# AgentFoundryExamples/lqr-quadcopter-test

Hardware: AMD Instinct MI355X
Metric: env-steps/sec at 65 536 parallel episodes per GPU (30 s @ dt=0.01, Riccati-LQR closed loop) (higher is better)
Workload: dtype f64; 1 GPU; BASELINE configs[1]: 65536 episodes/GPU x 3000 steps, linear target, Riccati-LQR shared K, RK4 dt=0.01; episodes_per_gpu=65536, episodes_total=65536, parallelism=episode-sharded x1

## Files before the change

lqr-quadcopter-test_amd/csrc/qt_device.hpp:

```cpp
#pragma once

#include <hip/hip_runtime.h>
#include <math.h>
#include <stdint.h>

#include "../../include/quadtrack.h"
#include "qt_glibc.hpp"
#include "qt_math.hpp"

namespace qt {

constexpr double kPi = 3.141592653589793;
constexpr double kTwoPi = 6.283185307179586;
constexpr double kMaxTilt = kPi / 3.0;

__device__ __forceinline__ double clipd(double v, double lo, double hi) {
  double r = v < lo ? lo : v;
  return r > hi ? hi : r;
}

__device__ __forceinline__ double dot3_blas(double a, double b, double c) { return fma(c, c, fma(b, b, a * a)); }
__device__ __forceinline__ double norm3(double a, double b, double c) { return sqrt(dot3_blas(a, b, c)); }

__device__ __forceinline__ bool same_sign(double a, double b) {
// ... 343 lines not shown
  double o[5];
  rk4_linear(delta, h, 1.0, zero, o);
  L.cv = o[3], L.pv = o[4];
  double sw = 0.0, sp = 0.0;
#pragma unroll
  for (int i = 0; i < 4; ++i) {
    double f[4] = {0.0, 0.0, 0.0, 0.0};
    f[i] = 1.0;
    rk4_linear(delta, h, 0.0, f, o);
    L.wv[i] = o[3];
    sw += o[3];
    if (i < 3) L.pa[i] = o[4], sp += o[4];
  }
  const double g = pl.gz * pl.inv_mass;
  L.gv = g * sw;
  L.gp = g * sp;
  return L;
}

struct Horizon {
  int on;
  double tmax;
  double vmax;
  double vmax2;
  double inv_2vmax;
  double vabs;
  double pmax;
  double pabs;
  double inv_dang;
  double inv_tstep;
  double slack;
  long long tie_exp_bits;
  int dual_below;
};

QT_HD Horizon make_horizon(const qt_env_params& e, const qt_ctrl_params& c, const RateLin& rl) {
  Horizon h{};
  const double tm = fmax(fabs(c.min_thrust), fabs(c.max_thrust));
  const bool ok = e.max_velocity > 1e-100 && e.max_velocity < 1e150 && e.max_position > 1e-100 &&
                  e.max_position < 1e150 && e.dt > 1e-100 && e.dt < 1e3 && fabs(e.max_episode_time) < 1e150 &&
                  tm < 1e150 && c.max_rate >= 0.0 && c.max_rate < 1e150;
  if (!ok) return h;
  h.on = 1;
  h.tmax = tm;
  h.vmax = e.max_velocity * (1.0 - 1e-12);
  h.vmax2 = h.vmax * h.vmax;
  h.inv_2vmax = 1.0 / (2.0 * h.vmax);
  h.vabs = e.max_velocity * 1e-14;
  h.pmax = e.max_position;
  h.pabs = e.max_position * 1e-15 + 1e-300;
  h.inv_dang = 1.0 / ((fabs(rl.ay) + fabs(rl.au)) * c.max_rate * (1.0 + 1e-9) + 2e-15);
  h.inv_tstep = 1.0 / ((e.dt + (fabs(e.max_episode_time) + e.dt) * 4.5e-16) * (1.0 + 1e-9));
  h.slack = 1.0 + 1e-9;
  {
    int q = 0;
    double m = frexp(e.dt, &q) * 9007199254740992.0;
    q -= 53;
    while (fmod(m, 2.0) == 0.0) m *= 0.5, ++q;
    const long long be = (long long)(q + 53) + 1023;
    h.tie_exp_bits = (be > 0 && be < 2047) ? (be << 52) : -1;
  }
  return h;
}

struct LaunchConst {
  RateLin rl;
  VelLin vl;
  Plant pl;
  Horizon hz;
  double rc[5][3], rs[5][3];
  double om[5][3];
  unsigned long long* defer_flag;
  unsigned long long epoch;
  double* reward;
  const double* fresh_off;
  double* met;
};

QT_HD int pattern_omegas(const qt_env_params& e, int motion, double* om) {
  if (motion == QT_MOTION_CIRCULAR) {
    om[0] = e.speed / e.radius;
    return 1;
  }
  if (motion == QT_MOTION_SINUSOIDAL) {
    om[0] = 2.0 * kPi * e.frequency;
    om[1] = 2.0 * kPi * (e.frequency * 1.3);
// ... 437 lines not shown
  return tl ? QT_TERM_TIME_LIMIT : (pb ? QT_TERM_POSITION_BOUNDS : QT_TERM_RUNNING);
}


template <int KC, bool KS>
struct Gains {
  static constexpr int kCount = KC == 3 ? 9 : (KS ? (KC == 9 ? 9 : 6) : 4 * KC);
  double k[kCount];
};

template <int KC>
__host__ __device__ constexpr int structured_index(int j) {
  constexpr int rows[9] = {0, 0, 1, 1, 2, 2, 0, 1, 2};
  constexpr int cols[9] = {2, 5, 1, 4, 0, 3, 8, 7, 6};
  return rows[j] * KC + cols[j];
}

struct FFLane {
  double vg[3], ag[3], vmax;
};

__host__ __device__ inline FFLane ff_uniform(const qt_ctrl_params& c) {
  if (!c.feedforward_enabled) return FFLane{{0.0, 0.0, 0.0}, {0.0, 0.0, 0.0}, INFINITY};
  return FFLane{{c.ff_velocity_gain[0], c.ff_velocity_gain[1], c.ff_velocity_gain[2]},
                {c.ff_acceleration_gain[0], c.ff_acceleration_gain[1], c.ff_acceleration_gain[2]},
                c.ff_max_velocity};
}

__device__ __forceinline__ double add_product_rn(double a, double b, double c) {
#pragma clang fp contract(off)
  return a + b * c;
}

template <int KC, bool FF, bool KS, bool FAST = false>
__device__ __forceinline__ bool compute_action(const qt_ctrl_params& c, const Gains<KC, KS>& G, double hover,
                                               const double* qp, const double* qv, const Target& tg,
                                               const FFLane& f, double* integ, double* u, double* diag = nullptr,
                                               double em_fast = 0.0) {
  double ep[3], ev[3], tv[3] = {tg.v[0], tg.v[1], tg.v[2]}, ffa[3] = {0, 0, 0}, ffv[3] = {0, 0, 0};
#pragma unroll
  for (int i = 0; i < 3; ++i) ep[i] = tg.p[i] - qp[i];
  if (FF) {
    double vm = norm3(tv[0], tv[1], tv[2]);
    if (vm > f.vmax) {
      double scl = f.vmax / vm;
#pragma unroll
      for (int i = 0; i < 3; ++i) tv[i] = tv[i] * scl;
    }
#pragma unroll
    for (int i = 0; i < 3; ++i) {
      ffv[i] = f.vg[i] * tv[i];
      tv[i] = (1.0 + f.vg[i]) * tv[i];
    }
    double ac[3] = {tg.a[0], tg.a[1], tg.a[2]};
    double am = norm3(ac[0], ac[1], ac[2]);
    if (am > c.ff_max_acceleration && am > 0) {
#pragma unroll
      for (int i = 0; i < 3; ++i) ac[i] = ac[i] / am * c.ff_max_acceleration;
    }
#pragma unroll
    for (int i = 0; i < 3; ++i) ffa[i] = f.ag[i] * ac[i];
  }
#pragma unroll
  for (int i = 0; i < 3; ++i) ev[i] = tv[i] - qv[i];
  const double s[6] = {ep[0], ep[1], ep[2], ev[0], ev[1], ev[2]};
  double uf[4];
  if (KC == 9) {
// ... 24 lines not shown
      uf[1] = (G.k[2] * s[1] + G.k[3] * s[4]) + G.k[7] * integ[1];
      uf[2] = (G.k[4] * s[0] + G.k[5] * s[3]) + G.k[8] * integ[0];
      uf[3] = 0.0;
    } else {
#pragma unroll
      for (int r = 0; r < 4; ++r) {
        double a = 0.0, b = 0.0;
#pragma unroll
        for (int j = 0; j < 6; ++j) a += G.k[r * KC + j] * s[j];
#pragma unroll
        for (int j = 0; j < 3; ++j) b += G.k[r * KC + 6 + j] * integ[j];
        uf[r] = a + b;
      }
    }
  } else if (KS) {
    uf[0] = G.k[0] * s[2] + G.k[1] * s[5];
    uf[1] = G.k[2] * s[1] + G.k[3] * s[4];
    uf[2] = G.k[4] * s[0] + G.k[5] * s[3];
    uf[3] = 0.0;
  } else {
#pragma unroll
    for (int r = 0; r < 4; ++r) {
      double a = 0.0;
#pragma unroll
      for (int j = 0; j < 6; ++j) a += G.k[r * KC + j] * s[j];
      uf[r] = a;
    }
  }
  const double raw0 = FF ? hover + uf[0] + ffa[2] : hover + uf[0];
  const double raw1 = FF ? uf[1] + -ffa[1] : uf[1];
  const double raw2 = FF ? uf[2] + ffa[0] : uf[2];
  const double raw3 = uf[3];
  u[0] = clip_num(raw0, c.min_thrust, c.max_thrust);
  u[1] = clip_num(raw1, -c.max_rate, c.max_rate);
  u[2] = clip_num(raw2, -c.max_rate, c.max_rate);
  u[3] = (KS && FAST) ? 0.0 : clip_num(raw3, -c.max_rate, c.max_rate);
  if (!FAST && any_lane(!isfinite((raw0 + raw1) + (raw2 + raw3)))) {
    u[0] = raw0 != raw0 ? raw0 : u[0];
    u[1] = raw1 != raw1 ? raw1 : u[1];
    u[2] = raw2 != raw2 ? raw2 : u[2];
    u[3] = raw3 != raw3 ? raw3 : u[3];
  }
  if (diag) {
#pragma unroll
    for (int i = 0; i < 6; ++i) diag[i] = s[i];
#pragma unroll
    for (int i = 0; i < 4; ++i) diag[6 + i] = uf[i];
#pragma unroll
    for (int i = 0; i < 3; ++i) diag[10 + i] = ffv[i], diag[13 + i] = ffa[i];
  }
  return (u[0] != raw0) || (u[1] != raw1) || (u[2] != raw2) || (u[3] != raw3);
}

template <bool FF, bool FAST = false>
__device__ __forceinline__ void compute_action_pid(const qt_ctrl_params& c, const double* g, double hover,
                                                   const double* qp, const double* qv, const Target& tg, double now,
                                                   const FFLane& f, double* integ, double* u,
                                                   double* diag = nullptr) {
  const double *kp = g, *ki = g + 3, *kd = g + 6;
  double ep[3], tv[3] = {tg.v[0], tg.v[1], tg.v[2]}, ffa[3] = {0, 0, 0}, ffv[3] = {0, 0, 0};
#pragma unroll
  for (int i = 0; i < 3; ++i) ep[i] = tg.p[i] - qp[i];
  const double last = integ[3];
  const bool none = (__double_as_longlong(last) & 0x7fffffffffffffffLL) > 0x7ff0000000000000LL;
  const double dt = none ? 0.0 : now - last;
  integ[3] = now;
  const double lim = c.integral_limit;
  if (FAST) {
// ... 64 lines not shown
```

lqr-quadcopter-test_amd/csrc/qt_kernels.hpp:

```cpp
#pragma once
#include <hip/hip_runtime.h>

#include <type_traits>

#include "qt_device.hpp"


#ifndef QT_ABLATE
#define QT_ABLATE 0
#endif
#define QT_ABL_METRICS 1
#define QT_ABL_CONSTRAIN 2
#define QT_ABL_TERMINATION 4
#define QT_ABL_CONTROLLER 8
#define QT_ABL_TARGET 16

#ifndef QT_CLOCK_STAMP
#define QT_CLOCK_STAMP 0
#endif

namespace qtk {

using namespace qt;

// ... 446 lines not shown
    if (ADVANCE) rotor_advance<QT_MOTION_CIRCULAR>(k, dtt, rs, rc);
    target_from_rotor<FF, QT_MOTION_CIRCULAR>(e, pt, rs, rc, tg);
  } else if (motion == QT_MOTION_FIGURE8 && !FF) {
    if (ADVANCE) rotor_advance<QT_MOTION_FIGURE8>(k, dtt, rs, rc);
    target_from_rotor<false, QT_MOTION_FIGURE8>(e, pt, rs, rc, tg);
  } else {
    target_state<FF, true>(e, motion, pt, t, tg);
  }
}

__device__ __forceinline__ void clamp_velocity(const qt_env_params& e, double* x) {
  const double s = dot3_blas(x[3], x[4], x[5]);
  if (norm_gt(s, e.max_velocity)) {
    const double vm = sqrt(s);
#pragma unroll
    for (int i = 3; i < 6; ++i) x[i] = x[i] / vm * e.max_velocity;
  }
}

__device__ __forceinline__ void tilt_clamp(double* x, Trig& ta) {
  double sm, cm;
  sincos_tilt(kMaxTilt, &sm, &cm);
#pragma unroll
  for (int i = 0; i < 2; ++i) {
    x[6 + i] = clip_num(x[6 + i], -kMaxTilt, kMaxTilt);
    ta.s[i] = clip_num(ta.s[i], -sm, sm);
    ta.c[i] = fmax(ta.c[i], cm);
  }
}

constexpr int kMaxHorizon = 62;
constexpr int kVotedBurst = 4;

template <bool TILT, bool BINADE>
__device__ __forceinline__ int yaw0_horizon(const qt_env_params& e, const Horizon& hz, const VelLin& lin,
                                            const Plant& pl, const double* x, double t, int rem) {
  const double tmi = hz.tmax * pl.inv_mass;
  const double sw = (fabs(lin.wv[0]) + fabs(lin.wv[1])) + (fabs(lin.wv[2]) + fabs(lin.wv[3]));
  const double spa = (fabs(lin.pa[0]) + fabs(lin.pa[1])) + fabs(lin.pa[2]);
  const double dv = fma(fma(tmi, sw, fabs(lin.gv)), hz.slack, hz.vabs);
  const double dp = fma(fma(fabs(lin.pv), hz.vmax, fma(tmi, spa, fabs(lin.gp))), hz.slack, hz.pabs);
  const double s = fma(x[5], x[5], fma(x[4], x[4], x[3] * x[3]));
  double h = (hz.vmax2 - s) * hz.inv_2vmax * __builtin_amdgcn_rcp(dv);
  h = fmin(h, (hz.pmax - fmax(fabs(x[0]), fmax(fabs(x[1]), fabs(x[2])))) * __builtin_amdgcn_rcp(dp));
  if (TILT) h = fmin(h, (kMaxTilt - fmax(fabs(x[6]), fabs(x[7]))) * hz.inv_dang);
  h = fmin(h, (e.max_episode_time - t) * hz.inv_tstep);
  bool bin_ok = true;
  if (BINADE) {
    const long long eb = __double_as_longlong(t) & 0x7ff0000000000000LL;
    h = fmin(h, (__longlong_as_double(eb + (1LL << 52)) - t) * hz.inv_tstep);
    bin_ok = t > 0.0 && eb != hz.tie_exp_bits;
  }
  h = fma(h, 1.0 - 1e-6, -1.0);
  const bool lane_ok = h >= 2.0 && lin.cv >= 0.0 && lin.cv <= 1.0 && bin_ok;
  const int hl = lane_ok ? (int)fmin(h, (double)kMaxHorizon) : 0;
  int H = 0;
#pragma unroll
  for (int bit = 32; bit >= 2; bit >>= 1)
    if (__builtin_amdgcn_ballot_w64(hl < H + bit) == 0) H += bit;
  const int rcap = (rem - 1) & ~1;
  return hz.on ? (H < rcap ? H : rcap) : 0;
}

constexpr int kDualBelow = 8;
#ifndef QT_GROUPED_DUAL
#define QT_GROUPED_DUAL 0
#endif

template <bool RIDE>
__device__ __forceinline__ void ride_target(const qt_env_params& e, bool still, Target& tg) {
  if constexpr (RIDE) {
#pragma unroll
    for (int i = 0; i < 3; ++i) {
      tg.p[i] = still ? e.center[i] : tg.p[i];
      tg.v[i] = still ? 0.0 : tg.v[i];
      tg.a[i] = still ? 0.0 : tg.a[i];
    }
  }
}

template <int MOTION, int KC, bool FF, bool KS, bool UNI, bool DUAL = false, bool RIDE = false>
__device__ __forceinline__ void run_yaw0(const qt_env_params& e, const qt_ctrl_params& c, const qt_criteria& cr,
                                         int motion, const Pattern& pt, const Plant& pl_lane, double hover,
                                         const Gains<KC, KS>& G, const FFLane& fl, double* x, double* integ,
                                         Target& tg, double& t, Acc& a, int nsteps, const LaunchConst& k,
                                         bool still = false) {
  constexpr bool kRotor = MOTION == QT_MOTION_CIRCULAR || MOTION == QT_MOTION_SINUSOIDAL ||
                          (MOTION == QT_MOTION_FIGURE8 && !FF);
  constexpr int kNeg = -(1 << 30);
  const Plant pl = UNI ? k.pl : pl_lane;
  const VelLin lin = UNI ? k.vl : make_vel_lin(e, pl_lane);
  const double R = cr.target_radius, eR = e.target_radius;
  const double vm2 = e.max_velocity * e.max_velocity * (1.0 - 1e-14);
  const double pos_up = nextafter(e.max_position, INFINITY);
  const int W = cr.overshoot_window;
  double rs[3] = {0.0, 0.0, 0.0}, rc[3] = {1.0, 1.0, 1.0};
  if constexpr (kRotor) {
    rotor_init<MOTION>(pt, t, rs, rc);
    target_from_rotor<FF, MOTION>(e, pt, rs, rc, tg);
  } else if constexpr (MOTION < 0) {
    rotor_init_rt<FF>(motion, pt, t, rs, rc);
    rotor_target_rt<FF, false>(e, k, motion, pt, t, 0.0, rs, rc, tg);
  } else {
    target_state<FF, true>(e, motion, pt, t, tg);
  }
  ride_target<RIDE>(e, still, tg);
  double err = sqrt_pos(sq3_ref(tg.p[0] - x[0], tg.p[1] - x[1], tg.p[2] - x[2]));
  Trig ta;
  trig_of<true>(x + 6, ta);
  int z = a.prev_on == 1 ? 1 : (a.os_streak >= 0 ? a.os_streak + 1 : kNeg);
  double cur = a.os_cur;
  int on_pre = a.on_pre, on_post = a.on_post, os_count = a.os_count;
  bool stepped = false;
  constexpr bool kTiltHorizon = KC != 9;
  constexpr bool kFold = kRotor && KC == 9;
  int s = 0;
  while (a.term == QT_TERM_RUNNING && s < nsteps) {
    const int s0 = s;
    int rem = nsteps - s0 > (1 << 29) ? (1 << 29) : nsteps - s0;
    RateCoef rk;
    auto step = [&](auto vote, auto clamp, const double* fc, const double* fs) -> bool {
      constexpr bool VOTE = decltype(vote)::value, CLAMP = decltype(clamp)::value;
      rk.pin();
      const double a0[2] = {x[6], x[7]};
      double u[4];
      if (QT_ABLATE & QT_ABL_CONTROLLER) {
        u[0] = hover, u[1] = u[2] = u[3] = 0.0;
      } else {
        if constexpr (KC == 3)
          compute_action_pid<FF, true>(c, G.k, hover, x, x + 3, tg, t, fl, integ, u);
        else
          compute_action<KC, FF, KS, true>(c, G, hover, x, x + 3, tg, fl, integ, u, nullptr, err);
      }
      if (!(QT_ABLATE & QT_ABL_METRICS)) {
        a.sum_e += err;
        a.sum_e2 = fma(err, err, a.sum_e2);
        a.max_e = fmax(a.max_e, err);
        const bool on = err <= R;
        on_pre += on;
        a.sum_u += sqrt_sum(fma(u[2], u[2], fma(u[1], u[1], u[0] * u[0])));
        const bool counted = on & (z > W);
        os_count += counted;
        a.os_max = counted ? fmax(a.os_max, cur) : a.os_max;
        cur = on ? err - R : fmax(cur, err - R);
        z = on ? 1 : z + 1;
      }
      double d4[2];
      Trig t4;
      integrate_yaw0(k.rl, lin, pl, ta, x, u, rk, d4, t4);
      const double t0 = t;
      t += e.dt;
      if (!(QT_ABLATE & QT_ABL_TARGET)) {
        if constexpr (kRotor) {
          if (VOTE || !kFold)
            rotor_advance<MOTION>(k, (t - t0) - e.dt, rs, rc);
          else
            rotor_turn<MOTION>(fc, fs, rs, rc);
          target_from_rotor<FF, MOTION>(e, pt, rs, rc, tg);
        } else if constexpr (MOTION < 0) {
          rotor_target_rt<FF, true>(e, k, motion, pt, t, (t - t0) - e.dt, rs, rc, tg);
        } else {
          target_state<FF, true>(e, motion, pt, t, tg);
        }
        ride_target<RIDE>(e, still, tg);
      }
      err = sqrt_pos(sq3_ref(x[0] - tg.p[0], x[1] - tg.p[1], x[2] - tg.p[2]));
      on_post += err <= eR;
      if (!(QT_ABLATE & QT_ABL_CONSTRAIN)) constrain_fast_apply<true>(e, x);
      attitude_trig_resid(x + 6, a0, d4, t4, ta);
      if ((VOTE || CLAMP || !kTiltHorizon) && !(QT_ABLATE & QT_ABL_CONSTRAIN)) tilt_clamp(x, ta);
      if constexpr (!VOTE) return false;
      --rem;
      double stop_m =
          fmax(fmax(fmax(fabs(x[0]), fmax(fabs(x[1]), fabs(x[2]))) - pos_up, (x[3] * x[3] + x[4] * x[4] + x[5] * x[5]) - vm2),
               fmax(t - e.max_episode_time, -(double)rem));
      return __builtin_amdgcn_ballot_w64(stop_m >= 0.0) != 0;
    };
    do {
      int H = yaw0_horizon<kTiltHorizon, kFold>(e, k.hz, lin, pl, x, t, rem);
      bool clamp_body = false;
      if constexpr (DUAL) {
        if (H < k.hz.dual_below) {
          const int H2 = yaw0_horizon<false, kFold>(e, k.hz, lin, pl, x, t, rem);
          if (H2 > H) H = H2, clamp_body = true;
        }
      }
      using F = std::false_type;
      using T = std::true_type;
      if constexpr (kFold) {
        double fc[3], fs[3];
        rotor_fold<MOTION>(k, ((t + e.dt) - t) - e.dt, fc, fs);
        for (int j = 4; j <= H; j += 4) {
          step(F{}, F{}, fc, fs);
          step(F{}, F{}, fc, fs);
          step(F{}, F{}, fc, fs);
          step(F{}, F{}, fc, fs);
        }
        if (H & 2) {
          step(F{}, F{}, fc, fs);
          step(F{}, F{}, fc, fs);
        }
      } else if (DUAL && clamp_body) {
        for (int j = 4; j <= H; j += 4) {
          step(F{}, T{}, nullptr, nullptr);
          step(F{}, T{}, nullptr, nullptr);
          step(F{}, T{}, nullptr, nullptr);
          step(F{}, T{}, nullptr, nullptr);
        }
        if (H & 2) {
          step(F{}, T{}, nullptr, nullptr);
          step(F{}, T{}, nullptr, nullptr);
        }
      } else {
        for (int j = 4; j <= H; j += 4) {
          step(F{}, F{}, nullptr, nullptr);
          step(F{}, F{}, nullptr, nullptr);
          step(F{}, F{}, nullptr, nullptr);
          step(F{}, F{}, nullptr, nullptr);
        }
        if (H & 2) {
          step(F{}, F{}, nullptr, nullptr);
          step(F{}, F{}, nullptr, nullptr);
        }
      }
      rem -= H;
      const int nv = H > 0 ? 0 : (k.hz.on ? kVotedBurst : (1 << 30));
      bool stop = false;
      for (int j = 0; j < nv && !stop; ++j) stop = step(std::true_type{}, std::false_type{}, nullptr, nullptr);
      if (stop) break;
    } while (true);
    const int ran = (nsteps - s0 > (1 << 29) ? (1 << 29) : nsteps - s0) - rem;
    s += ran;
    a.steps += ran;
    stepped = true;
    z = z <= 0 ? kNeg : z;
    if (!(QT_ABLATE & QT_ABL_CONSTRAIN)) clamp_velocity(e, x);
    a.term = (QT_ABLATE & QT_ABL_TERMINATION) ? (t >= e.max_episode_time ? QT_TERM_TIME_LIMIT : QT_TERM_RUNNING)
                                               : termination_fast(e, t, x);
  }
  if (stepped) {
    a.on_pre = on_pre, a.on_post = on_post, a.os_count = os_count;
    a.prev_on = z == 1 ? 1 : 0;
    a.os_streak = z >= 2 ? z - 1 : -1;
    a.os_cur = cur;
  }
}

template <int FLAVOR, int MOTION, int KC, bool FF, bool KS, bool UNI = false, bool FRESH = true, bool REC = true,
          int INTEG = -1, bool RIDE = false, bool PIN = true>
__device__ __forceinline__ void rollout_lane(const qt_env_params& e, const qt_ctrl_params& c, const qt_criteria& cr,
                                             const BatchDev& b, const qt_state& st, int nsteps,
                                             double* __restrict__ rec, int deferred, const LaunchConst& lc,
                                             int64_t slot) {
  const int64_t n = b.n, ep = episode_of(b, slot);
  const int motion = MOTION >= 0 ? MOTION : motion_of(b, e, ep);
  const bool still = RIDE && slot_motion(b, slot) == QT_MOTION_STATIONARY;
  Pattern pt = pattern_of(b, e, motion, ep);
  if (RIDE) pt.c0 = still ? 0.0 : pt.c0, pt.c1 = still ? 0.0 : pt.c1, pt.c2 = still ? 0.0 : pt.c2;
  const Plant pl = UNI ? lc.pl : make_plant(e, b.plant_mass ? b.plant_mass[ep] : e.mass);
  const double hover = UNI ? c.hover_thrust : (b.hover ? b.hover[ep] : c.hover_thrust);
  Gains<KC, KS> G;
  load_gains<KC, KS, UNI>(b, ep, G);
  const FFLane fl = FF ? ff_of(b, c, ep) : FFLane{};

  constexpr int NI = KC == 9 ? 3 : (KC == 3 ? 4 : 0);
  double x[12], integ[4] = {0, 0, 0, 0};
  Target tg;
  double t;
  Acc a;
  if (FRESH && lc.fresh_off) {
    target_state<true>(e, motion, pt, 0.0, tg);
#pragma unroll
    for (int i = 0; i < 3; ++i) x[i] = tg.p[i] + lc.fresh_off[i * n + ep];
#pragma unroll
    for (int i = 3; i < 12; ++i) x[i] = 0.0;
    if (KC == 3) integ[3] = __longlong_as_double(0x7ff8000000000000LL);
    t = 0.0;
    a = Acc{0, 0, -INFINITY, 0, 0, 0, 0, 0, 0, -1, -1, 0, 0, QT_TERM_RUNNING};
  } else {
#pragma unroll
    for (int i = 0; i < 12; ++i) x[i] = st.x[i * n + ep];
#pragma unroll
// ... 23 lines not shown
      st.target[(6 + i) * n + ep] = tg.a[i];
    }
    st.t[ep] = t;
    store_acc(st.acc, n, ep, a);
  };

  bool lane_ok = a.term != QT_TERM_RUNNING ||
                 (all_finite(G.k, Gains<KC, KS>::kCount) && all_finite(x, 12) && all_finite(integ, 3) &&
                  all_finite(tg.p, 3) && all_finite(tg.v, 3) && all_finite(tg.a, 3) && finite_bits(hover) &&
                  (!FF || (all_finite(fl.vg, 3) && all_finite(fl.ag, 3) && !(fl.vmax < 0.0))) &&
                  finite_bits(pl.inv_mass) && finite_bits(t) && fabs(t) < 1e300);
  for (int i = 9; i < 12; ++i) lane_ok = lane_ok && fabs(x[i]) <= e.max_angular_velocity;
  if (FLAVOR == kExact && b.nseg && b.motion) lane_ok = lane_ok && (int)b.motion[ep] == slot_motion(b, slot);
  if (b.seg_check >= 0 && b.motion) lane_ok = lane_ok && (int)b.motion[ep] == b.seg_check;
  if (FLAVOR == kYaw0 || deferred == kYaw0)
    lane_ok = lane_ok && x[8] == 0.0 && x[11] == 0.0 && fabs(x[6]) <= kMaxTilt && fabs(x[7]) <= kMaxTilt &&
              fabs(x[9]) <= c.max_rate && fabs(x[10]) <= c.max_rate;
  const bool wave_ok = __builtin_amdgcn_ballot_w64(!lane_ok) == 0;
  if (FLAVOR != kExact) {
    if (!wave_ok) {
      if (lc.defer_flag) *lc.defer_flag = lc.epoch;
      if (FRESH && lc.fresh_off) store_state();
      return;
    }
    const bool rw = FRESH && lc.reward && a.term == QT_TERM_RUNNING;
    if (rw) lc.reward[ep] += a.sum_e + sqrt_pos(sq3_ref(tg.p[0] - x[0], tg.p[1] - x[1], tg.p[2] - x[2]));
#if QT_CLOCK_STAMP && defined(QT_FAST_TU)
    const unsigned long long t0 = __builtin_amdgcn_s_memtime(), r0 = __builtin_amdgcn_s_memrealtime();
#endif
    if constexpr (FLAVOR == kYaw0)
      run_yaw0<MOTION, KC, FF, KS, UNI,
               (FRESH || QT_GROUPED_DUAL) && KC != 9 &&
                   (MOTION == QT_MOTION_CIRCULAR || MOTION == QT_MOTION_SINUSOIDAL || MOTION == QT_MOTION_FIGURE8),
               RIDE>(e, c, cr, motion, pt, pl, hover, G, fl, x, integ, tg, t, a, nsteps, lc, still);
    else
      run_steps<true, MOTION, KC, FF, KS>(e, c, cr, motion, pt, pl, hover, G, fl, x, integ, tg, t, a, nsteps, rec,
                                          n, ep);
#if QT_CLOCK_STAMP && defined(QT_FAST_TU)
    const unsigned long long t1 = __builtin_amdgcn_s_memtime(), r1 = __builtin_amdgcn_s_memrealtime();
    const int64_t wave = ((int64_t)blockIdx.x * kBlock + threadIdx.x) >> 6;
    if ((threadIdx.x & 63) == 0 && wave < kStampWaves) {
      g_qt_stamps[wave][0] = t0, g_qt_stamps[wave][1] = t1;
      g_qt_stamps[wave][2] = r0, g_qt_stamps[wave][3] = r1;
      g_qt_stamps[wave][4] = (unsigned)__builtin_amdgcn_s_getreg((31 << 11) | 4);
      g_qt_stamps[wave][5] = (unsigned)__builtin_amdgcn_s_getreg((15 << 11) | 20);
    }
#endif
    if (rw) {
      const double q0 = x[0] - tg.p[0], q1 = x[1] - tg.p[1], q2 = x[2] - tg.p[2];
      lc.reward[ep] -= a.sum_e + sqrt_pos(sq3_ref(q0, q1, q2));
      lc.reward[n + ep] = sqrt(dot3_blas(q0, q1, q2));
    }
  } else {
    if (deferred != kExact && wave_ok) return;
    run_steps<false, MOTION, KC, FF, KS, INTEG, PIN>(e, c, cr, motion, pt, pl, hover, G, fl, x, integ, tg, t, a, nsteps,
                                         REC ? rec : nullptr, n, ep, REC ? lc.reward : nullptr);
  }
  if (!FF && (motion == QT_MOTION_CIRCULAR || motion == QT_MOTION_SINUSOIDAL || motion == QT_MOTION_FIGURE8)) {
    Target full;
    target_state<true>(e, motion, pt, t, full);
#pragma unroll
    for (int i = 0; i < 3; ++i) tg.a[i] = still ? 0.0 : full.a[i];
  }

  store_state();
  if (FRESH && lc.met) store_metrics(cr, a, t, lc.met, n, ep);
}

template <int FLAVOR, int MOTION, int KC, bool FF, bool KS, bool UNI = false, bool REC = true, int INTEG = -1,
          bool PIN = true>
__global__ __launch_bounds__(kBlock) void rollout_kernel(qt_env_params e, qt_ctrl_params c, qt_criteria cr,
                                                         BatchDev b, qt_state st, int nsteps,
                                                         double* __restrict__ rec, int deferred, LaunchConst lc) {
  if (FLAVOR == kExact && deferred != kExact && lc.defer_flag && *lc.defer_flag != lc.epoch) return;
  const int64_t slot = slot_at(b, (int64_t)blockIdx.x * kBlock + threadIdx.x);
  if (slot < 0) return;
  rollout_lane<FLAVOR, MOTION, KC, FF, KS, UNI, true, REC, INTEG, false, PIN>(e, c, cr, b, st, nsteps, rec, deferred, lc,
                                                                             slot);
}

#ifndef QT_GROUPED_WAVES
#define QT_GROUPED_WAVES 2
#endif
#ifndef QT_GROUPED_RIDERS
#define QT_GROUPED_RIDERS 1
#endif
template <int KC, bool FF, bool KS>
__global__ __launch_bounds__(kBlock) __attribute__((amdgpu_waves_per_eu(QT_GROUPED_WAVES))) void rollout_grouped_kernel(qt_env_params e, qt_ctrl_params c, qt_criteria cr,
                                                                 BatchDev b, qt_state st, int nsteps, LaunchConst lc) {
  const int64_t p = (int64_t)blockIdx.x * kBlock + threadIdx.x;
  bool ride;
  const int64_t slot = slot_at(b, p, ride);
  if (slot < 0) return;
  const int wm = wave_motion(b, p);
  if (b.motion && __builtin_amdgcn_ballot_w64((int)b.motion[episode_of(b, slot)] != slot_motion(b, slot)) != 0) {
    if (lc.defer_flag) *lc.defer_flag = lc.epoch;
    return;
  }
  const int key = wm + ((QT_GROUPED_RIDERS && __builtin_amdgcn_ballot_w64(ride) != 0) ? 8 : 0);
  switch (key) {
    case QT_MOTION_STATIONARY:
      rollout_lane<kYaw0, QT_MOTION_STATIONARY, KC, FF, KS, false, false>(e, c, cr, b, st, nsteps, nullptr, kExact, lc, slot);
      break;
    case QT_MOTION_LINEAR:
      rollout_lane<kYaw0, QT_MOTION_LINEAR, KC, FF, KS, false, false>(e, c, cr, b, st, nsteps, nullptr, kExact, lc, slot);
      break;
    case QT_MOTION_CIRCULAR:
      rollout_lane<kYaw0, QT_MOTION_CIRCULAR, KC, FF, KS, false, false>(e, c, cr, b, st, nsteps, nullptr, kExact, lc, slot);
      break;
    case QT_MOTION_SINUSOIDAL:
      rollout_lane<kYaw0, QT_MOTION_SINUSOIDAL, KC, FF, KS, false, false>(e, c, cr, b, st, nsteps, nullptr, kExact, lc, slot);
// ... 14 lines not shown
      rollout_lane<kYaw0, QT_MOTION_SINUSOIDAL, KC, FF, KS, false, false, true, -1, true>(e, c, cr, b, st, nsteps,
                                                                                       nullptr, kExact, lc, slot);
      break;
    case 8 + QT_MOTION_FIGURE8:
      rollout_lane<kYaw0, QT_MOTION_FIGURE8, KC, FF, KS, false, false, true, -1, true>(e, c, cr, b, st, nsteps, nullptr,
                                                                                    kExact, lc, slot);
      break;
#endif
    default:
      break;
  }
}

inline BatchDev to_dev(const qt_batch* b) {
  BatchDev d{};
  d.n = b->n, d.motion = b->motion, d.pattern = b->pattern, d.plant_mass = b->plant_mass;
  d.hover = b->hover_thrust, d.K = b->K, d.k_cols = b->k_cols, d.k_per_episode = b->k_per_episode;
  d.order = b->order, d.ff = b->ff, d.slot0 = 0, d.slot_end = b->n;
  d.nseg = 0;
  d.seg_check = -1;
  return d;
}

inline int grid_of(int64_t n) { return (int)((n + kBlock - 1) / kBlock); }

inline int check_launch() { return hipGetLastError() == hipSuccess ? QT_OK : QT_ELAUNCH; }

inline bool valid_state(const qt_state& st, bool need_integ) {
  return st.x && st.t && st.acc && st.target && (!need_integ || st.integ);
}

void launch_fast(int flavor, bool uni, bool grouped, int kc, bool ff, bool ks, int motion, int grid, hipStream_t s,
                 const qt_env_params& e, const qt_ctrl_params& c, const qt_criteria& cr, const BatchDev& b,
                 const qt_state& st, int nsteps, const LaunchConst& lc);

void launch_pair(int motion, int grid, hipStream_t s, const qt_env_params& e, const qt_ctrl_params& c,
                 const qt_criteria& cr, const BatchDev& b, const qt_state& st, int nsteps, const LaunchConst& lc);

template <class L, int KC, bool FF, bool KS, class... A>
void dispatch_motion(int motion, A&&... args) {
  switch (motion) {
    case QT_MOTION_STATIONARY: L::template run<QT_MOTION_STATIONARY, KC, FF, KS>(args...); break;
    case QT_MOTION_LINEAR: L::template run<QT_MOTION_LINEAR, KC, FF, KS>(args...); break;
    case QT_MOTION_CIRCULAR: L::template run<QT_MOTION_CIRCULAR, KC, FF, KS>(args...); break;
    case QT_MOTION_SINUSOIDAL: L::template run<QT_MOTION_SINUSOIDAL, KC, FF, KS>(args...); break;
    case QT_MOTION_FIGURE8: L::template run<QT_MOTION_FIGURE8, KC, FF, KS>(args...); break;
    default: L::template run<-1, KC, FF, KS>(args...);
  }
}

template <class L, int KC, class... A>
void dispatch_ffks(bool ff, bool ks, int motion, A&&... args) {
  if constexpr (KC == 3) {
    if (ff) dispatch_motion<L, 3, true, true>(motion, args...);
    else dispatch_motion<L, 3, false, true>(motion, args...);
  } else if (ff) {
    if (ks) dispatch_motion<L, KC, true, true>(motion, args...);
    else dispatch_motion<L, KC, true, false>(motion, args...);
  } else {
    if (ks) dispatch_motion<L, KC, false, true>(motion, args...);
    else dispatch_motion<L, KC, false, false>(motion, args...);
  }
}

template <class L, class... A>
void dispatch_rollout(int kc, bool ff, bool ks, int motion, A&&... args) {
  if (kc == 9) dispatch_ffks<L, 9>(ff, ks, motion, args...);
// ... 7 lines not shown
```

lqr-quadcopter-test_amd/csrc/qt_rollout.hip:

```cpp
#include "qt_kernels.hpp"
#include <atomic>
#include <cstring>
#include <map>
#include <mutex>

using namespace qtk;

namespace {


__global__ __launch_bounds__(kBlock) void reset_kernel(qt_env_params e, BatchDev b, const double* __restrict__ off,
                                                       qt_state st) {
  const int64_t slot = (int64_t)blockIdx.x * kBlock + threadIdx.x;
  if (slot >= b.n) return;
  const int64_t n = b.n, ep = episode_of(b, slot);
  const int motion = motion_of(b, e, ep);
  const Pattern pt = pattern_of(b, e, motion, ep);
  Target tg;
  target_state<true>(e, motion, pt, 0.0, tg);
#pragma unroll
  for (int i = 0; i < 3; ++i) st.x[i * n + ep] = tg.p[i] + off[i * n + ep];
#pragma unroll
  for (int i = 3; i < 12; ++i) st.x[i * n + ep] = 0.0;
  if (st.integ) {
// ... 514 lines not shown

unsigned long long* defer_flag_for(hipStream_t s) {
  static std::mutex mu;
  static std::map<std::pair<int, hipStream_t>, unsigned long long*> flags;
  int dev = 0;
  if (hipGetDevice(&dev) != hipSuccess) return nullptr;
  std::lock_guard<std::mutex> lock(mu);
  auto it = flags.find({dev, s});
  if (it != flags.end()) return it->second;
  unsigned long long* f = nullptr;
  if (hipMalloc(&f, sizeof(*f)) != hipSuccess) return nullptr;
  if (hipMemsetAsync(f, 0, sizeof(*f), s) != hipSuccess) {
    (void)hipFree(f);
    return nullptr;
  }
  flags[{dev, s}] = f;
  return f;
}

int dual_below() {
  const char* s = getenv("QT_DUAL_BELOW");
  if (!s || !*s) return kDualBelow;
  char* end = nullptr;
  const long x = strtol(s, &end, 10);
  if (*end != '\0' || x < 0 || x > 62) {
    static std::atomic<bool> warned{false};
    if (!warned.exchange(true))
      fprintf(stderr, "quadtrack: ignoring QT_DUAL_BELOW=%s (not a whole number in 0..62)\n", s);
    return kDualBelow;
  }
  return (int)x;
}

bool pair_on() {
  const char* s = getenv("QT_PAIR");
  return !(s && s[0] == '0' && s[1] == '\0');
}

bool pair_fits(int kc, bool ff, bool ks, bool grouped, int motion, const BatchDev& b, const LaunchConst& lc) {
  return pair_on() && !grouped && kc == 6 && ks && !ff && !b.plant_mass && !b.hover && !lc.reward &&
         motion >= QT_MOTION_STATIONARY && motion <= QT_MOTION_FIGURE8 && b.nseg == 0 && !b.order &&
         b.seg_check < 0 && b.slot0 == 0 && b.slot_end == b.n && b.n > 0 && 2 * b.n <= ExactLaunch::pin_lanes();
}

int flavor_for(int kc, bool ks, bool no_yaw, const qt_env_params& e, const qt_ctrl_params& c, const double* rec) {
  const bool fast = QT_ABLATE == 0 && rec == nullptr && fast_path_ok(e, c);
  if (fast && (ks || kc == 3 || no_yaw) && rate_bounded_ok(e, c)) return kYaw0;
  if (QT_ABLATE == 0 && rec == nullptr && (ks || kc == 3 || no_yaw) && euler_yaw0_ok(e, c)) return kYaw0;
  return fast ? kFast : kExact;
}

bool riders_on() {
  const char* s = getenv("QT_RIDERS");
  return !(s && s[0] == '0' && s[1] == '\0');
}

int64_t grouped_waves(BatchDev& bg, bool riders) {
  int stat = -1;
  for (int i = 0; i < bg.nseg; ++i)
    if (bg.seg_motion[i] == QT_MOTION_STATIONARY && stat < 0) stat = i;
  if (riders && stat >= 0) {
    int64_t next = bg.seg_lo[stat], avail = bg.seg_end[stat] - bg.seg_lo[stat];
    for (int i = 0; i < bg.nseg; ++i) {
      if (i == stat) continue;
      const int64_t gap = (64 - (bg.seg_end[i] - bg.seg_lo[i]) % 64) % 64;
      const int64_t take = gap < avail ? gap : avail;
      bg.ride_lo[i] = next, bg.ride_cnt[i] = take;
      next += take, avail -= take;
    }
    bg.seg_lo[stat] = next;
  }
  int64_t waves = 0;
  for (int i = 0; i < bg.nseg; ++i) {
    waves += (bg.seg_end[i] - bg.seg_lo[i] + bg.ride_cnt[i] + 63) / 64;
    bg.wave_end[i] = waves;
  }
  return waves;
}

int launch_rollout(int kc, bool ff, bool ks, bool no_yaw, int motion, int grid, hipStream_t s, const qt_env_params& e,
                   const qt_ctrl_params& c, const qt_criteria& cr, const BatchDev& b, const qt_state& st, int nsteps,
                   double* rec, bool grouped = false, double* reward = nullptr, const double* fresh_off = nullptr,
                   double* met = nullptr, int exact_motion = -2) {
  if (exact_motion == -2) exact_motion = motion;
  LaunchConst lc = make_launch_const(e);
  lc.hz = make_horizon(e, c, lc.rl);
  lc.hz.dual_below = dual_below();
  lc.reward = reward;
  lc.fresh_off = fresh_off, lc.met = met;
  const bool ks_eff = ks || kc == 3;
  const bool uni = !b.plant_mass && !b.hover && !b.k_per_episode;
  const int flavor = flavor_for(kc, ks, no_yaw, e, c, rec);
  if (flavor != kExact) {
    lc.defer_flag = defer_flag_for(s);
    lc.epoch = g_defer_epoch.fetch_add(1, std::memory_order_relaxed) + 1;
    if (flavor == kYaw0 && pair_fits(kc, ff, ks, grouped, motion, b, lc))
      launch_pair(motion, (int)((2 * b.n + kBlock - 1) / kBlock), s, e, c, cr, b, st, nsteps, lc);
    else
      launch_fast(flavor, uni, grouped, kc, ff, ks_eff, motion, grid, s, e, c, cr, b, st, nsteps, lc);
    if (hipGetLastError() != hipSuccess) return QT_ELAUNCH;
    lc.fresh_off = nullptr;
  }
  dispatch_rollout<ExactLaunch>(kc, ff, ks_eff, grouped ? -1 : exact_motion, flavor, grid, s, e, c, cr, b, st, nsteps,
                                rec, lc);
  return check_launch();
}

int rollout_batch(const qt_env_params& e, const qt_ctrl_params& c, const qt_criteria& cr, const qt_batch* batch,
                  qt_state st, int nsteps, double* rec, int32_t nseg, const int32_t* seg_motion,
                  const int64_t* seg_end, hipStream_t s, const double* fresh_off = nullptr, double* met = nullptr) {
  BatchDev b = to_dev(batch);
  const bool ff = c.feedforward_enabled != 0 || batch->ff != nullptr;
  const bool ks = batch->k_structured != 0;
  const bool no_yaw = batch->k_no_yaw != 0;
  if (nseg == 0)
    return launch_rollout(batch->k_cols, ff, ks, no_yaw, batch->motion ? -1 : e.motion, grid_of(batch->n), s, e, c,
                          cr, b, st, nsteps, rec, false, nullptr, fresh_off, met);
  bool mixed = false;
  for (int32_t i = 0; i < nseg; ++i) mixed = mixed || seg_motion[i] < 0;
  if (!mixed && flavor_for(batch->k_cols, ks, no_yaw, e, c, rec) == kYaw0) {
    BatchDev bg = b;
    int64_t prev_end = 0;
    bool fits = true;
    for (int32_t i = 0; i < nseg && fits; ++i) {
      const int64_t cnt = seg_end[i] - prev_end;
      if (cnt > 0) {
        if (bg.nseg == 8) {
          fits = false;
          break;
        }
        bg.seg_motion[bg.nseg] = (int8_t)seg_motion[i];
        bg.seg_lo[bg.nseg] = prev_end;
// ... 226 lines not shown
```

lqr-quadcopter-test_amd/csrc/qt_rollout_fast.hip:

```cpp
#define QT_FAST_TU 1
#include <hip/hip_runtime.h>

#ifndef QT_CLOCK_STAMP
#define QT_CLOCK_STAMP 0
#endif
#if QT_CLOCK_STAMP
constexpr int kStampWaves = 1 << 16;
__device__ unsigned long long g_qt_stamps[kStampWaves][6];
#endif

#include "qt_kernels.hpp"
#include "qt_pair.hpp"

namespace qtk {

namespace {
struct FastLaunch {
  template <int MOTION, int KC, bool FF, bool KS>
  static void run(int flavor, bool uni, int grid, hipStream_t s, const qt_env_params& e, const qt_ctrl_params& c,
                  const qt_criteria& cr, const BatchDev& b, const qt_state& st, int nsteps, const LaunchConst& lc) {
    (void)uni;
    if (flavor == kYaw0)
      rollout_kernel<kYaw0, MOTION, KC, FF, KS><<<grid, kBlock, 0, s>>>(e, c, cr, b, st, nsteps, nullptr, kExact, lc);
    else
      rollout_kernel<kFast, MOTION, KC, FF, KS><<<grid, kBlock, 0, s>>>(e, c, cr, b, st, nsteps, nullptr, kExact, lc);
  }
};
}

struct GroupedLaunch {
  template <int MOTION, int KC, bool FF, bool KS>
  static void run(int grid, hipStream_t s, const qt_env_params& e, const qt_ctrl_params& c, const qt_criteria& cr,
                  const BatchDev& b, const qt_state& st, int nsteps, const LaunchConst& lc) {
    if constexpr (MOTION == -1)
      rollout_grouped_kernel<KC, FF, KS><<<grid, kBlock, 0, s>>>(e, c, cr, b, st, nsteps, lc);
  }
};

void launch_fast(int flavor, bool uni, bool grouped, int kc, bool ff, bool ks, int motion, int grid, hipStream_t s,
                 const qt_env_params& e, const qt_ctrl_params& c, const qt_criteria& cr, const BatchDev& b,
                 const qt_state& st, int nsteps, const LaunchConst& lc) {
  if (grouped && flavor == kYaw0)
    dispatch_rollout<GroupedLaunch>(kc, ff, ks, -1, grid, s, e, c, cr, b, st, nsteps, lc);
  else
    dispatch_rollout<FastLaunch>(kc, ff, ks, motion, flavor, uni, grid, s, e, c, cr, b, st, nsteps, lc);
}

namespace {
template <int MOTION>
void launch_pair_motion(int grid, hipStream_t s, const qt_env_params& e, const qt_ctrl_params& c,
                        const qt_criteria& cr, const BatchDev& b, const qt_state& st, int nsteps,
                        const LaunchConst& lc) {
  if (b.k_per_episode)
    rollout_pair_kernel<MOTION, true><<<grid, kBlock, 0, s>>>(e, c, cr, b, st, nsteps, lc);
  else
    rollout_pair_kernel<MOTION, false><<<grid, kBlock, 0, s>>>(e, c, cr, b, st, nsteps, lc);
}
}

void launch_pair(int motion, int grid, hipStream_t s, const qt_env_params& e, const qt_ctrl_params& c,
                 const qt_criteria& cr, const BatchDev& b, const qt_state& st, int nsteps, const LaunchConst& lc) {
  switch (motion) {
    case QT_MOTION_LINEAR: launch_pair_motion<QT_MOTION_LINEAR>(grid, s, e, c, cr, b, st, nsteps, lc); break;
    case QT_MOTION_CIRCULAR: launch_pair_motion<QT_MOTION_CIRCULAR>(grid, s, e, c, cr, b, st, nsteps, lc); break;
    case QT_MOTION_SINUSOIDAL: launch_pair_motion<QT_MOTION_SINUSOIDAL>(grid, s, e, c, cr, b, st, nsteps, lc); break;
    case QT_MOTION_FIGURE8: launch_pair_motion<QT_MOTION_FIGURE8>(grid, s, e, c, cr, b, st, nsteps, lc); break;
    default: launch_pair_motion<QT_MOTION_STATIONARY>(grid, s, e, c, cr, b, st, nsteps, lc); break;
  }
}

}

#if QT_CLOCK_STAMP
extern "C" {
int qt_debug_stamps(unsigned long long* out, int64_t waves) {
  if (!out || waves < 0 || waves > kStampWaves) return QT_EINVAL;
  return hipMemcpyFromSymbol(out, HIP_SYMBOL(g_qt_stamps), sizeof(unsigned long long) * 6 * waves) == hipSuccess
             ? QT_OK
// ... 5 lines not shown
```

Baseline: 147.4 billion env-steps/s.

## Add rate-saturation horizon to skip rate clipping in yaw0 fast bursts

Adds a per-lane bound on how many steps the LQR rate commands provably stay under max_rate, folds it into the yaw0 burst horizon, and compiles the non-voting step with rate clipping removed for 6-gain, non-feedforward, stationary or linear targets. Also adds an EQR kernel variant, used when the criteria radius equals the env target radius, that derives the on-target counter from per-burst bookkeeping, and rewrites the overshoot max update without a select. The intent is to shorten the per-step dependency chain inside bursts. In exchange the horizon computation costs more per burst and shorter horizons may cause more frequent re-evaluation, and the change adds new kernel instantiations.

```diff
diff --git a/lqr-quadcopter-test_amd/csrc/qt_device.hpp b/lqr-quadcopter-test_amd/csrc/qt_device.hpp
--- a/lqr-quadcopter-test_amd/csrc/qt_device.hpp
+++ b/lqr-quadcopter-test_amd/csrc/qt_device.hpp
@@ -399,6 +399,9 @@
   double slack;
   long long tie_exp_bits;
   int dual_below;
+  int rate_on;
+  double rate_lim;
+  double tstep;
 };
 
 QT_HD Horizon make_horizon(const qt_env_params& e, const qt_ctrl_params& c, const RateLin& rl) {
@@ -419,6 +422,9 @@
   h.inv_dang = 1.0 / ((fabs(rl.ay) + fabs(rl.au)) * c.max_rate * (1.0 + 1e-9) + 2e-15);
   h.inv_tstep = 1.0 / ((e.dt + (fabs(e.max_episode_time) + e.dt) * 4.5e-16) * (1.0 + 1e-9));
   h.slack = 1.0 + 1e-9;
+  h.rate_on = 1;
+  h.rate_lim = c.max_rate * (1.0 - 1e-9);
+  h.tstep = (e.dt + (fabs(e.max_episode_time) + e.dt) * 4.5e-16) * (1.0 + 1e-9);
   {
     int q = 0;
     double m = frexp(e.dt, &q) * 9007199254740992.0;
@@ -922,7 +928,7 @@
   return a + b * c;
 }
 
-template <int KC, bool FF, bool KS, bool FAST = false>
+template <int KC, bool FF, bool KS, bool FAST = false, bool NORATE = false>
 __device__ __forceinline__ bool compute_action(const qt_ctrl_params& c, const Gains<KC, KS>& G, double hover,
                                                const double* qp, const double* qv, const Target& tg,
                                                const FFLane& f, double* integ, double* u, double* diag = nullptr,
@@ -1013,8 +1019,8 @@
   const double raw2 = FF ? uf[2] + ffa[0] : uf[2];
   const double raw3 = uf[3];
   u[0] = clip_num(raw0, c.min_thrust, c.max_thrust);
-  u[1] = clip_num(raw1, -c.max_rate, c.max_rate);
-  u[2] = clip_num(raw2, -c.max_rate, c.max_rate);
+  u[1] = NORATE ? raw1 : clip_num(raw1, -c.max_rate, c.max_rate);
+  u[2] = NORATE ? raw2 : clip_num(raw2, -c.max_rate, c.max_rate);
   u[3] = (KS && FAST) ? 0.0 : clip_num(raw3, -c.max_rate, c.max_rate);
   if (!FAST && any_lane(!isfinite((raw0 + raw1) + (raw2 + raw3)))) {
     u[0] = raw0 != raw0 ? raw0 : u[0];
diff --git a/lqr-quadcopter-test_amd/csrc/qt_kernels.hpp b/lqr-quadcopter-test_amd/csrc/qt_kernels.hpp
--- a/lqr-quadcopter-test_amd/csrc/qt_kernels.hpp
+++ b/lqr-quadcopter-test_amd/csrc/qt_kernels.hpp
@@ -502,9 +502,51 @@
 constexpr int kMaxHorizon = 62;
 constexpr int kVotedBurst = 4;
 
-template <bool TILT, bool BINADE>
+template <int KC, bool KS>
+__device__ __forceinline__ double rate_distance(const Horizon& hz, const VelLin& lin, const Plant& pl,
+                                                const Gains<KC, KS>& G, const Target& tg, const double* x) {
+  static_assert(KC == 6, "6-column gains");
+  const double tmi = hz.tmax * pl.inv_mass;
+  const double sw = (fabs(lin.wv[0]) + fabs(lin.wv[1])) + (fabs(lin.wv[2]) + fabs(lin.wv[3]));
+  const double spa = (fabs(lin.pa[0]) + fabs(lin.pa[1])) + fabs(lin.pa[2]);
+  const double dp = fma(fma(fabs(lin.pv), hz.vmax, fma(tmi, spa, fabs(lin.gp))), hz.slack, hz.pabs);
+  const double dvc = fma(fma(1.0 - lin.cv, hz.vmax, fma(tmi, sw, fabs(lin.gv))), hz.slack, hz.vabs);
+  double one = 1.0;
+  asm volatile("" : "+v"(one));
+  double s[6], d[6];
+#pragma unroll
+  for (int j = 0; j < 3; ++j) {
+    s[j] = fabs(tg.p[j] - x[j]);
+    s[3 + j] = fabs(tg.v[j] - x[3 + j]);
+    d[j] = fma(fabs(tg.v[j]), hz.tstep, dp + hz.pabs) * one;
+    d[3 + j] = dvc * one;
+  }
+  double h = INFINITY;
+#pragma unroll
+  for (int r = 1; r <= 2; ++r) {
+    double num = hz.rate_lim, den = 1e-300;
+    if constexpr (KS) {
+      const int j = r == 1 ? 1 : 0;
+      const double kp = fabs(G.k[2 * r]), kv = fabs(G.k[2 * r + 1]);
+      num = fma(-kv, s[3 + j], fma(-kp, s[j], num));
+      den = fma(kv, d[3 + j], fma(kp, d[j], den));
+    } else {
+#pragma unroll
+      for (int j = 0; j < 6; ++j) {
+        const double ka = fabs(G.k[r * KC + j]);
+        num = fma(-ka, s[j], num);
+        den = fma(ka, d[j], den);
+      }
+    }
+    h = fmin(h, num * __builtin_amdgcn_rcp(den));
+  }
+  return hz.rate_on ? h : 0.0;
+}
+
+template <bool TILT, bool BINADE, bool RATE = false>
 __device__ __forceinline__ int yaw0_horizon(const qt_env_params& e, const Horizon& hz, const VelLin& lin,
-                                            const Plant& pl, const double* x, double t, int rem) {
+                                            const Plant& pl, const double* x, double t, int rem,
+                                            double h_more = 0.0) {
   const double tmi = hz.tmax * pl.inv_mass;
   const double sw = (fabs(lin.wv[0]) + fabs(lin.wv[1])) + (fabs(lin.wv[2]) + fabs(lin.wv[3]));
   const double spa = (fabs(lin.pa[0]) + fabs(lin.pa[1])) + fabs(lin.pa[2]);
@@ -515,6 +557,7 @@
   h = fmin(h, (hz.pmax - fmax(fabs(x[0]), fmax(fabs(x[1]), fabs(x[2])))) * __builtin_amdgcn_rcp(dp));
   if (TILT) h = fmin(h, (kMaxTilt - fmax(fabs(x[6]), fabs(x[7]))) * hz.inv_dang);
   h = fmin(h, (e.max_episode_time - t) * hz.inv_tstep);
+  if constexpr (RATE) h = fmin(h, h_more);
   bool bin_ok = true;
   if (BINADE) {
     const long long eb = __double_as_longlong(t) & 0x7ff0000000000000LL;
@@ -549,7 +592,7 @@
   }
 }
 
-template <int MOTION, int KC, bool FF, bool KS, bool UNI, bool DUAL = false, bool RIDE = false>
+template <int MOTION, int KC, bool FF, bool KS, bool UNI, bool DUAL = false, bool RIDE = false, bool EQR = false>
 __device__ __forceinline__ void run_yaw0(const qt_env_params& e, const qt_ctrl_params& c, const qt_criteria& cr,
                                          int motion, const Pattern& pt, const Plant& pl_lane, double hover,
                                          const Gains<KC, KS>& G, const FFLane& fl, double* x, double* integ,
@@ -584,10 +627,13 @@
   bool stepped = false;
   constexpr bool kTiltHorizon = KC != 9;
   constexpr bool kFold = kRotor && KC == 9;
+  constexpr bool kRate = KC == 6 && !FF && (MOTION == QT_MOTION_STATIONARY || MOTION == QT_MOTION_LINEAR);
+  constexpr bool kEqr = EQR && !(QT_ABLATE & QT_ABL_METRICS);
   int s = 0;
   while (a.term == QT_TERM_RUNNING && s < nsteps) {
     const int s0 = s;
     int rem = nsteps - s0 > (1 << 29) ? (1 << 29) : nsteps - s0;
+    if constexpr (kEqr) on_post -= on_pre + (int)(err <= R);
     RateCoef rk;
     auto step = [&](auto vote, auto clamp, const double* fc, const double* fs) -> bool {
       constexpr bool VOTE = decltype(vote)::value, CLAMP = decltype(clamp)::value;
@@ -600,7 +646,7 @@
         if constexpr (KC == 3)
           compute_action_pid<FF, true>(c, G.k, hover, x, x + 3, tg, t, fl, integ, u);
         else
-          compute_action<KC, FF, KS, true>(c, G, hover, x, x + 3, tg, fl, integ, u, nullptr, err);
+          compute_action<KC, FF, KS, true, kRate && !VOTE>(c, G, hover, x, x + 3, tg, fl, integ, u, nullptr, err);
       }
       if (!(QT_ABLATE & QT_ABL_METRICS)) {
         a.sum_e += err;
@@ -612,7 +658,7 @@
         const bool counted = on & (z > W);
         os_count += counted;
         a.os_max = counted ? fmax(a.os_max, cur) : a.os_max;
-        cur = on ? err - R : fmax(cur, err - R);
+        cur = fmax(__hiloint2double(on ? (int)0xffefffff : __double2hiint(cur), __double2loint(cur)), err - R);
         z = on ? 1 : z + 1;
       }
       double d4[2];
@@ -635,7 +681,7 @@
         ride_target<RIDE>(e, still, tg);
       }
       err = sqrt_pos(sq3_ref(x[0] - tg.p[0], x[1] - tg.p[1], x[2] - tg.p[2]));
-      on_post += err <= eR;
+      if constexpr (!kEqr) on_post += err <= eR;
       if (!(QT_ABLATE & QT_ABL_CONSTRAIN)) constrain_fast_apply<true>(e, x);
       attitude_trig_resid(x + 6, a0, d4, t4, ta);
       if ((VOTE || CLAMP || !kTiltHorizon) && !(QT_ABLATE & QT_ABL_CONSTRAIN)) tilt_clamp(x, ta);
@@ -647,11 +693,13 @@
       return __builtin_amdgcn_ballot_w64(stop_m >= 0.0) != 0;
     };
     do {
-      int H = yaw0_horizon<kTiltHorizon, kFold>(e, k.hz, lin, pl, x, t, rem);
+      double hr = 0.0;
+      if constexpr (kRate) hr = rate_distance<KC, KS>(k.hz, lin, pl, G, tg, x);
+      int H = yaw0_horizon<kTiltHorizon, kFold, kRate>(e, k.hz, lin, pl, x, t, rem, hr);
       bool clamp_body = false;
       if constexpr (DUAL) {
         if (H < k.hz.dual_below) {
-          const int H2 = yaw0_horizon<false, kFold>(e, k.hz, lin, pl, x, t, rem);
+          const int H2 = yaw0_horizon<false, kFold, kRate>(e, k.hz, lin, pl, x, t, rem, hr);
           if (H2 > H) H = H2, clamp_body = true;
         }
       }
@@ -702,6 +750,7 @@
     const int ran = (nsteps - s0 > (1 << 29) ? (1 << 29) : nsteps - s0) - rem;
     s += ran;
     a.steps += ran;
+    if constexpr (kEqr) on_post += on_pre + (int)(err <= R);
     stepped = true;
     z = z <= 0 ? kNeg : z;
     if (!(QT_ABLATE & QT_ABL_CONSTRAIN)) clamp_velocity(e, x);
@@ -717,7 +766,7 @@
 }
 
 template <int FLAVOR, int MOTION, int KC, bool FF, bool KS, bool UNI = false, bool FRESH = true, bool REC = true,
-          int INTEG = -1, bool RIDE = false, bool PIN = true>
+          int INTEG = -1, bool RIDE = false, bool PIN = true, bool EQR = false>
 __device__ __forceinline__ void rollout_lane(const qt_env_params& e, const qt_ctrl_params& c, const qt_criteria& cr,
                                              const BatchDev& b, const qt_state& st, int nsteps,
                                              double* __restrict__ rec, int deferred, const LaunchConst& lc,
@@ -807,7 +856,7 @@
       run_yaw0<MOTION, KC, FF, KS, UNI,
                (FRESH || QT_GROUPED_DUAL) && KC != 9 &&
                    (MOTION == QT_MOTION_CIRCULAR || MOTION == QT_MOTION_SINUSOIDAL || MOTION == QT_MOTION_FIGURE8),
-               RIDE>(e, c, cr, motion, pt, pl, hover, G, fl, x, integ, tg, t, a, nsteps, lc, still);
+               RIDE, EQR>(e, c, cr, motion, pt, pl, hover, G, fl, x, integ, tg, t, a, nsteps, lc, still);
     else
       run_steps<true, MOTION, KC, FF, KS>(e, c, cr, motion, pt, pl, hover, G, fl, x, integ, tg, t, a, nsteps, rec,
                                           n, ep);
@@ -843,15 +892,15 @@
 }
 
 template <int FLAVOR, int MOTION, int KC, bool FF, bool KS, bool UNI = false, bool REC = true, int INTEG = -1,
-          bool PIN = true>
+          bool PIN = true, bool EQR = false>
 __global__ __launch_bounds__(kBlock) void rollout_kernel(qt_env_params e, qt_ctrl_params c, qt_criteria cr,
                                                          BatchDev b, qt_state st, int nsteps,
                                                          double* __restrict__ rec, int deferred, LaunchConst lc) {
   if (FLAVOR == kExact && deferred != kExact && lc.defer_flag && *lc.defer_flag != lc.epoch) return;
   const int64_t slot = slot_at(b, (int64_t)blockIdx.x * kBlock + threadIdx.x);
   if (slot < 0) return;
-  rollout_lane<FLAVOR, MOTION, KC, FF, KS, UNI, true, REC, INTEG, false, PIN>(e, c, cr, b, st, nsteps, rec, deferred, lc,
-                                                                             slot);
+  rollout_lane<FLAVOR, MOTION, KC, FF, KS, UNI, true, REC, INTEG, false, PIN, EQR>(e, c, cr, b, st, nsteps, rec,
+                                                                                  deferred, lc, slot);
 }
 
 #ifndef QT_GROUPED_WAVES
@@ -932,7 +981,7 @@
 
 void launch_fast(int flavor, bool uni, bool grouped, int kc, bool ff, bool ks, int motion, int grid, hipStream_t s,
                  const qt_env_params& e, const qt_ctrl_params& c, const qt_criteria& cr, const BatchDev& b,
-                 const qt_state& st, int nsteps, const LaunchConst& lc);
+                 const qt_state& st, int nsteps, const LaunchConst& lc, bool eqr);
 
 void launch_pair(int motion, int grid, hipStream_t s, const qt_env_params& e, const qt_ctrl_params& c,
                  const qt_criteria& cr, const BatchDev& b, const qt_state& st, int nsteps, const LaunchConst& lc);
diff --git a/lqr-quadcopter-test_amd/csrc/qt_rollout.hip b/lqr-quadcopter-test_amd/csrc/qt_rollout.hip
--- a/lqr-quadcopter-test_amd/csrc/qt_rollout.hip
+++ b/lqr-quadcopter-test_amd/csrc/qt_rollout.hip
@@ -570,6 +570,15 @@
   return (int)x;
 }
 
+int rate_horizon_on() {
+  const char* s = getenv("QT_RATE_HORIZON");
+  if (!s || !*s) return 1;
+  if ((s[0] == '0' || s[0] == '1') && s[1] == '\0') return s[0] == '1';
+  static std::atomic<bool> warned{false};
+  if (!warned.exchange(true)) fprintf(stderr, "quadtrack: ignoring QT_RATE_HORIZON=%s (not 0 or 1)\n", s);
+  return 1;
+}
+
 bool pair_on() {
   const char* s = getenv("QT_PAIR");
   return !(s && s[0] == '0' && s[1] == '\0');
@@ -624,6 +633,8 @@
   LaunchConst lc = make_launch_const(e);
   lc.hz = make_horizon(e, c, lc.rl);
   lc.hz.dual_below = dual_below();
+  lc.hz.rate_on = lc.hz.on ? rate_horizon_on() : 0;
+  const bool eqr = memcmp(&cr.target_radius, &e.target_radius, sizeof(double)) == 0;
   lc.reward = reward;
   lc.fresh_off = fresh_off, lc.met = met;
   const bool ks_eff = ks || kc == 3;
@@ -635,7 +646,7 @@
     if (flavor == kYaw0 && pair_fits(kc, ff, ks, grouped, motion, b, lc))
       launch_pair(motion, (int)((2 * b.n + kBlock - 1) / kBlock), s, e, c, cr, b, st, nsteps, lc);
     else
-      launch_fast(flavor, uni, grouped, kc, ff, ks_eff, motion, grid, s, e, c, cr, b, st, nsteps, lc);
+      launch_fast(flavor, uni, grouped, kc, ff, ks_eff, motion, grid, s, e, c, cr, b, st, nsteps, lc, eqr);
     if (hipGetLastError() != hipSuccess) return QT_ELAUNCH;
     lc.fresh_off = nullptr;
   }
diff --git a/lqr-quadcopter-test_amd/csrc/qt_rollout_fast.hip b/lqr-quadcopter-test_amd/csrc/qt_rollout_fast.hip
--- a/lqr-quadcopter-test_amd/csrc/qt_rollout_fast.hip
+++ b/lqr-quadcopter-test_amd/csrc/qt_rollout_fast.hip
@@ -17,9 +17,17 @@
 namespace {
 struct FastLaunch {
   template <int MOTION, int KC, bool FF, bool KS>
-  static void run(int flavor, bool uni, int grid, hipStream_t s, const qt_env_params& e, const qt_ctrl_params& c,
-                  const qt_criteria& cr, const BatchDev& b, const qt_state& st, int nsteps, const LaunchConst& lc) {
+  static void run(int flavor, bool uni, bool eqr, int grid, hipStream_t s, const qt_env_params& e,
+                  const qt_ctrl_params& c, const qt_criteria& cr, const BatchDev& b, const qt_state& st, int nsteps,
+                  const LaunchConst& lc) {
     (void)uni;
+    if constexpr (KC == 6 && !FF && (MOTION == QT_MOTION_STATIONARY || MOTION == QT_MOTION_LINEAR)) {
+      if (flavor == kYaw0 && eqr) {
+        rollout_kernel<kYaw0, MOTION, KC, FF, KS, false, true, -1, true, true><<<grid, kBlock, 0, s>>>(
+            e, c, cr, b, st, nsteps, nullptr, kExact, lc);
+        return;
+      }
+    }
     if (flavor == kYaw0)
       rollout_kernel<kYaw0, MOTION, KC, FF, KS><<<grid, kBlock, 0, s>>>(e, c, cr, b, st, nsteps, nullptr, kExact, lc);
     else
@@ -39,11 +47,11 @@
 
 void launch_fast(int flavor, bool uni, bool grouped, int kc, bool ff, bool ks, int motion, int grid, hipStream_t s,
                  const qt_env_params& e, const qt_ctrl_params& c, const qt_criteria& cr, const BatchDev& b,
-                 const qt_state& st, int nsteps, const LaunchConst& lc) {
+                 const qt_state& st, int nsteps, const LaunchConst& lc, bool eqr) {
   if (grouped && flavor == kYaw0)
     dispatch_rollout<GroupedLaunch>(kc, ff, ks, -1, grid, s, e, c, cr, b, st, nsteps, lc);
   else
-    dispatch_rollout<FastLaunch>(kc, ff, ks, motion, flavor, uni, grid, s, e, c, cr, b, st, nsteps, lc);
+    dispatch_rollout<FastLaunch>(kc, ff, ks, motion, flavor, uni, eqr, grid, s, e, c, cr, b, st, nsteps, lc);
 }
 
 namespace {
```

Result: faster. 151.0 billion env-steps/s, median of 6 (+2.4%).
